# konrad-kaminski/ratelimit

Hardware: AMD Instinct MI355X
Metric: rate-limit decisions/sec (whole node) at 10M/1B keys; p99 batch latency (higher is better)
Workload: dtype u32

## Files before the change

### ratelimit_amd/csrc/rl_engine.h

```cpp
#pragma once

#include <hip/hip_runtime.h>

#include <string>

#include "../../include/ratelimit_hip.h"
#include "rl_device.h"
#include "rl_kernels.h"
#include "rl_match.h"

namespace rl {

#ifndef RL_NBUF
#define RL_NBUF 4
#endif
constexpr uint32_t NBUF = RL_NBUF;
constexpr uint32_t ERRB_RING = 2 * NBUF;
constexpr uint32_t ERRW_B0 = NBUF + 3, ERRW_WORDS = ERRW_B0 + ERRB_RING;
constexpr uint32_t PROF_RING = 8;
constexpr uint32_t PROGRESS_RING = 64;

struct HostSlot {
  uint8_t* stem = nullptr;
  uint32_t *off = nullptr, *req = nullptr, *limit = nullptr, *hits = nullptr, *rule = nullptr;
// ... 82 lines not shown
  uint32_t *d_off = nullptr, *d_req = nullptr, *d_limit = nullptr, *d_hits = nullptr, *d_rule = nullptr;
  int64_t* d_now = nullptr;
  uint8_t *d_unit = nullptr, *d_flags = nullptr, *d_code = nullptr, *d_status = nullptr;
  uint32_t *d_rem = nullptr, *d_reset = nullptr;
  unsigned long long* d_stats = nullptr;
  uint32_t* h_err = nullptr;
  uint32_t* h_long = nullptr;
  uint32_t long_recent = 0;
  int long_mode = 1;
  uint32_t* h_big = nullptr;
  uint32_t big_recent = 0;
  int big_mode = 1;
  uint32_t* h_late = nullptr;
  uint32_t late_recent = 0;
  int late_mode = 1;
  unsigned long long* h_counters = nullptr;
  std::string last_error;
  uint64_t batches = 0, decisions = 0;
  bool prof = false;
  uint32_t prof_every = 1, prof_skip = 0;
  bool prof_pending[PROF_RING] = {};
  uint32_t prof_next = 0;
  hipEvent_t ev[PROF_RING][RL_NUM_STAGES + 1] = {};
  double stage_ms[RL_NUM_STAGES] = {};
  uint64_t prof_batches = 0;
  unsigned long long* d_kt_acc = nullptr;
  double wclk_khz = 0;
  uint8_t* cfg_blob = nullptr;
  CfgDev cfg_dev{};
  bool cfg_loaded = false;
// ... 97 lines not shown
```

### ratelimit_amd/csrc/rl_engine.hip

```cpp
#include <hip/hip_runtime.h>
#include <hip/hip_ext.h>

#include <algorithm>
#include <chrono>
#include <cstdio>
#include <cstdlib>
#include <random>
#include <cstring>
#include <string>
#include <vector>

#include "../../include/ratelimit_hip.h"
#include "rl_device.h"
#include "rl_kernels.h"
#include "rl_match.h"
#include "rl_engine.h"

using namespace rl;



namespace {

thread_local std::string g_err;
// ... 130 lines not shown
    big_full = c->big_recent > 0;
    if (c->big_recent) c->big_recent--;
  }
  uint32_t* bhint = c->big_mode == 1 ? c->h_big + k : nullptr;
  bool late_full = c->late_mode == 0;
  if (c->late_mode == 1) {
    for (uint32_t j = 0; j < NBUF; j++)
      if (__atomic_load_n(&c->h_late[j], __ATOMIC_RELAXED)) {
        __atomic_store_n(&c->h_late[j], 0u, __ATOMIC_RELAXED);
        c->late_recent = 4 * NBUF;
      }
    late_full = c->late_recent > 0;
    if (c->late_recent) c->late_recent--;
  }
  uint32_t* lhint = c->late_mode == 1 ? c->h_late + k : nullptr;
  if (pipelined) {
    hipStream_t a = c->pipe[k];
    hipEvent_t* ev = prof_events(c);
    (void)hipStreamWaitEvent(a, c->b_done[k], 0);
    (void)hipStreamWaitEvent(a, c->consumed[k], 0);
    launch_stage_a(b, c->s[k], isolate, P.per_second, a, ev, hint, lng, bhint, big_full);
    if (early) launch_b_begin_early(b, o, c->s[k], restore, a, c->log_ctr);
    (void)hipStreamWaitEvent(a, c->b_table[c->last], 0);
    launch_stage_b(b, o, t, P, c->s[k], restore, a, ev, errb_prev, c->b_table[k], ev ? c->d_kt_acc : nullptr,
                   early, lhint, late_full);
    (void)hipEventRecord(c->b_done[k], a);
  } else {
    if (!st) st = c->stream;
    (void)after_batches(c, st);
    hipEvent_t* ev = prof_events(c);
    launch_stage_a(b, c->s[k], isolate, P.per_second, st, ev, hint, lng, bhint, big_full);
    if (early) launch_b_begin_early(b, o, c->s[k], restore, st, c->log_ctr);
    launch_stage_b(b, o, t, P, c->s[k], restore, st, ev, errb_prev, c->b_table[k], ev ? c->d_kt_acc : nullptr,
                   early, lhint, late_full);
    (void)hipEventRecord(c->b_done[k], st);
  }
  c->last = k;
  return k;
}

hipError_t track(Engine* c, hipStream_t st) {
  if (c->seq_sub - c->seq_done >= PROGRESS_RING) {
    const hipError_t e = hipEventSynchronize(c->done_ring[c->seq_done % PROGRESS_RING]);
    if (e != hipSuccess) return e;
    c->seq_done++;
  }
  const hipError_t e = hipEventRecord(c->done_ring[c->seq_sub % PROGRESS_RING], st);
  c->seq_sub++;
  return e;
// ... 254 lines not shown
  ok = ok && dalloc(&c->d_code, n) == hipSuccess && dalloc(&c->d_status, n) == hipSuccess &&
       dalloc(&c->d_rem, n) == hipSuccess &&
       dalloc(&c->d_reset, n) == hipSuccess;
  ok = ok && dalloc(&c->d_stats, (size_t)cfg.max_rules * RL_NUM_STATS) == hipSuccess;
  ok = ok && hipHostMalloc((void**)&c->h_err, ERRW_WORDS * sizeof(uint32_t)) == hipSuccess;
  ok = ok && hipHostMalloc((void**)&c->h_counters, 8 * sizeof(unsigned long long)) == hipSuccess;
  ok = ok && hipHostMalloc((void**)&c->h_long, NBUF * sizeof(uint32_t)) == hipSuccess;
  if (ok) memset(c->h_long, 0, NBUF * sizeof(uint32_t));
  if (const char* sl = getenv("RL_SPLIT_LONG")) c->long_mode = atoi(sl);
  ok = ok && hipHostMalloc((void**)&c->h_big, NBUF * sizeof(uint32_t)) == hipSuccess;
  if (ok) memset(c->h_big, 0, NBUF * sizeof(uint32_t));
  if (const char* bc = getenv("RL_BIG_CUE")) c->big_mode = atoi(bc);
  ok = ok && hipHostMalloc((void**)&c->h_late, NBUF * sizeof(uint32_t)) == hipSuccess;
  if (ok) memset(c->h_late, 0, NBUF * sizeof(uint32_t));
  if (const char* lc = getenv("RL_LATE_CUE")) c->late_mode = atoi(lc);
  if (!ok) return fail("gpu: device allocation failed (table_slots/arena/max_batch too large?)", c);
  ok = hipMemsetAsync(c->slots, 0, c->nslots * sizeof(Slot), c->stream) == hipSuccess &&
       hipMemsetAsync(c->log_ctr, 0, (size_t)(LOG_PARTS + 1) * LOG_CTR_STRIDE * 8, c->stream) == hipSuccess &&
       hipMemsetAsync(c->errw, 0, ERRW_WORDS * 4, c->stream) == hipSuccess &&
       hipMemsetAsync(s0.time_floor, 0, 8, c->stream) == hipSuccess &&
       hipMemsetAsync(s0.counters, 0, 64, c->stream) == hipSuccess &&
       hipMemsetAsync(c->s[0].stripes, 0, (size_t)STAT_STRIPES * STAT_LDS_RULES * RL_NUM_STATS * 8, c->stream) ==
           hipSuccess &&
       hipMemsetAsync(c->d_stem, 0, (size_t)cfg.max_stem_bytes + 64, c->stream) == hipSuccess &&
       hipStreamSynchronize(c->stream) == hipSuccess;
  for (uint32_t k = 0; k < NBUF; k++)
    ok = ok && hipEventRecord(c->b_done[k], c->stream) == hipSuccess &&
         hipEventRecord(c->b_table[k], c->stream) == hipSuccess &&
         (k == 0 || hipMemsetAsync(c->s[k].stripes, 0, (size_t)STAT_STRIPES * STAT_LDS_RULES * RL_NUM_STATS * 8,
                                   c->stream) == hipSuccess) &&
// ... 72 lines not shown
  if (c->h_base) (void)hipHostFree(c->h_base);
  const Scratch& s0 = c->s[0];
  void* bufs[] = {c->slots, c->log, c->log_ctr, c->tear, c->arena, c->arena2, c->errw, s0.stripes, s0.time_floor, s0.counters, c->d_stem, c->d_off,
                  c->d_now, c->d_req, c->d_unit, c->d_flags, c->d_limit, c->d_hits, c->d_rule, c->d_code, c->d_status,
                  c->d_rem,
                  c->d_reset, c->d_stats};
  for (void* p : bufs)
    if (p) (void)hipFree(p);
  for (uint32_t k = 1; k < NBUF; k++)
    if (c->s[k].stripes) (void)hipFree(c->s[k].stripes);
  if (c->h_err) (void)hipHostFree(c->h_err);
  if (c->h_counters) (void)hipHostFree(c->h_counters);
  if (c->h_long) (void)hipHostFree(c->h_long);
  if (c->h_big) (void)hipHostFree(c->h_big);
  if (c->h_late) (void)hipHostFree(c->h_late);
  for (void* p : {(void*)c->cfg_blob, (void*)c->mbuf})
    if (p) (void)hipFree(p);
  if (c->h_match) (void)hipHostFree(c->h_match);
  for (uint32_t k = 0; k < NBUF; k++)
    if (c->pipe[k]) (void)hipStreamDestroy(c->pipe[k]);
  delete c;
}

int eng_do_limit_async(Engine* c, const rl_batch* in, rl_result* out, void* stream) {
  if (!c || !in || !out) return set_err(c, RL_E_INVALID, "gpu: null argument");
  RQ_SETTLE(c);
  int rc = check_sizes(c, in, 0);
  if (rc) return rc;
  if ((uintptr_t)in->stem_bytes & 3u) return set_err(c, RL_E_INVALID, "gpu: stem_bytes must be 4-byte aligned");
  HIPCHK(c, hipSetDevice(c->cfg.device));
// ... 2189 lines not shown
```

### ratelimit_amd/csrc/rl_kernels.h

```cpp
#pragma once

#include <hip/hip_runtime.h>
#include <stdint.h>

#include "rl_device.h"

namespace rl {

#ifndef RL_PART_ITEMS
#define RL_PART_ITEMS 16
#endif
constexpr uint32_t PART_ITEMS = RL_PART_ITEMS, PART_TILE = 256 * PART_ITEMS;
constexpr uint32_t PART_BITS = 10, PART_DIGITS = 1u << PART_BITS;
#ifndef RL_BIG_BLOCKS
#define RL_BIG_BLOCKS 64
#endif
constexpr uint32_t BIG_BLOCKS = RL_BIG_BLOCKS;
constexpr uint32_t BIG_ITEM_BLOCKS = 256;
constexpr uint32_t BIG_HEAVY = 4;

struct BigMeta {
  uint32_t d, S, base, nchunks, item0, r, rb_heavy, db_heavy;
  uint32_t heavy[BIG_HEAVY];
};
// ... 176 lines not shown
  uint32_t* errb;
  uint32_t* errs;
  int64_t* time_floor;
  unsigned long long* counters;
  uint32_t* route_start;
  uint8_t* route_dest;
  unsigned long long* route_hash;
  uint32_t* route_hist;
  unsigned long long* r_base;
  uint32_t* woff;
  unsigned long long* wtsum;
};

void launch_stage_a(const BatchDev& b, const Scratch& s, int isolate, int per_second, hipStream_t st,
                    hipEvent_t* ev = nullptr, uint32_t* long_hint = nullptr, bool long_kernel = false,
                    uint32_t* big_hint = nullptr, bool big_full = true);
void launch_stage_b(const BatchDev& b, const OutDev& o, const TableDev& t, const Params& P, const Scratch& s,
                    int restore, hipStream_t st, hipEvent_t* ev, const uint32_t* errb_prev, hipEvent_t table_done,
                    unsigned long long* kt_acc = nullptr, bool early = false, uint32_t* late_hint = nullptr,
                    bool late_full = true);
void launch_b_begin_early(const BatchDev& b, const OutDev& o, const Scratch& s, int restore, hipStream_t st,
                          const unsigned long long* log_ctr);
void launch_unpack(const rl_batch_compact& cb, const uint8_t* buf, uint32_t* req, uint8_t* unit, uint8_t* flags,
                   uint32_t* limit, uint32_t* hits, uint32_t* rule, int64_t* now, uint32_t* err, hipStream_t st);
void launch_unpack_range(const rl_batch_compact& cb, const uint8_t* buf, uint32_t d0, uint32_t d1, uint32_t q0,
                         uint32_t q1, uint32_t* req, uint8_t* unit, uint8_t* flags, uint32_t* limit, uint32_t* hits,
                         uint32_t* rule, int64_t* now, uint32_t* err, hipStream_t st);
constexpr uint32_t TO_HOST_MAX = 6;
struct ToHost {
  const uint8_t* src[TO_HOST_MAX];
  uint8_t* dst[TO_HOST_MAX];
  uint64_t bytes[TO_HOST_MAX];
  uint32_t n;
};
void launch_to_host(const ToHost& c, hipStream_t st);
// ... 73 lines not shown
```

### ratelimit_amd/csrc/rl_kernels.hip

```cpp
#include <hip/hip_runtime.h>
#include <stdint.h>
#include <cstdlib>

#include "rl_device.h"
#include "rl_kernels.h"

#ifndef RL_ABL
#define RL_ABL 0
#endif

namespace rl {

constexpr uint32_t HASH_LDS_BYTES = 16384;

__global__ __launch_bounds__(256) void k_prepare(BatchDev b, Rec* __restrict__ rec, uint32_t* __restrict__ keys,
                                                 uint32_t* err, uint32_t* errs, int isolate,
                                                 const int64_t* time_floor, uint32_t* defer_n,
                                                 uint32_t* big_n, uint32_t* work_n, uint32_t* __restrict__ run_flags,
                                                 unsigned long long* num_runs, uint32_t* __restrict__ hit_a,
                                                 unsigned long long* __restrict__ res, uint32_t* sorted_n,
                                                 uint32_t* uniq_n) {
  __shared__ uint32_t lds[HASH_LDS_BYTES / 4 + 4];
  const uint32_t tid = threadIdx.x;
  const uint32_t i = blockIdx.x * 256 + tid;
// ... 1575 lines not shown
      }
    }
    __syncthreads();
#pragma unroll
    for (uint32_t i = 0; i < B::ITEMS; i++) {
      const uint32_t p = strip0 + i * 64 + lane;
      if (p < n) {
        kk[i] = L.k[p];
        vv[i] = L.v[p];
        hh[i] = L.h[p];
      }
    }
  }
}

template <typename B, bool FROM_LDS>
__device__ inline void bucket_segment(BucketLds<B>& L, uint32_t d, uint32_t S, uint32_t base,
                                      const uint32_t* __restrict__ sk, const uint32_t* __restrict__ sh,
                                      uint32_t* __restrict__ segsum, uint32_t* __restrict__ rid,
                                      uint32_t* __restrict__ run_start, uint32_t* __restrict__ run_end,
                                      unsigned long long* num_runs, uint32_t* __restrict__ drun) {
  constexpr uint32_t IT = B::ITEMS;
  const uint32_t tid = threadIdx.x, lane = tid & 63, wave = tid >> 6;
  auto key = [&](uint32_t p) -> uint32_t { return FROM_LDS ? L.k[p] : sk[base + p]; };
  auto hit = [&](uint32_t p) -> uint32_t { return FROM_LDS ? L.h[p] : sh[base + p]; };
  uint32_t nh = 0, nd = 0;
  for (uint32_t c0 = 0; c0 < S; c0 += B::CAP) {
    uint32_t a[IT], b[IT], c[IT];
#pragma unroll
    for (uint32_t i = 0; i < IT; i++) {
      const uint32_t p = min(c0 + i * B::THREADS + tid, S - 1);
      a[i] = key(p ? p - 1 : 0);
      b[i] = key(p);
      c[i] = key(p > 1 ? p - 2 : 0);
    }
#pragma unroll
    for (uint32_t i = 0; i < IT; i++) {
      const uint32_t p = c0 + i * B::THREADS + tid;
      nh += (p < S && (p == 0 || a[i] != b[i])) ? 1u : 0u;
      nd += (p < S && p >= 1 && a[i] == b[i] && (p == 1 || c[i] != a[i])) ? 1u : 0u;
    }
  }
  nh = block_sum(L, nh);
  nd = block_sum(L, nd);
  BK_STAMP(d, 4);
  if (tid == 0) {
    const unsigned long long old = atomicAdd(num_runs, ((unsigned long long)nd << 32) | nh);
    L.rb = (uint32_t)old;
    L.db = (uint32_t)(old >> 32);
    L.dcnt = 0;
    L.nruns = nh;
    L.carry = SegPair{0, 0};
    L.hcarry = 0;
  }
  __syncthreads();
  const uint32_t rb = L.rb;
  for (uint32_t c0 = 0; c0 < S; c0 += B::CAP) {
    const uint32_t s0 = c0 + wave * B::STRIP;
    const uint32_t ni = s0 >= S ? 0u : min(IT, (S - s0 + 63) / 64);
    SegChunk ch[IT];
    SegPair agg{0, 0};
    uint32_t hc = 0;
    uint32_t kp[IT], kq[IT], hq[IT], kpp[IT];
#pragma unroll
    for (uint32_t j = 0; j < IT; j++) {
      const uint32_t q = min(s0 + 64 * j + lane, S - 1);
      kp[j] = key(q ? q - 1 : 0);
      kq[j] = key(q);
      hq[j] = hit(q);
      kpp[j] = key(q > 1 ? q - 2 : 0);
// ... 107 lines not shown
      const uint32_t y = __shfl_up(incl, o, 64);
      if (lane >= o) incl += y;
    }
    uint32_t rank = incl - nc;
#pragma unroll
    for (uint32_t i = 0; i < R; i++)
      if (first[i] && cnt[i] >= BK_HEAVY_MIN) {
        if (rank < BK_HEAVY) L.heavy[rank] = ks[i];
        rank++;
      }
    if (lane == 63) L.nheavy = min(incl, BK_HEAVY);
  }
  __syncthreads();
}

__global__ __launch_bounds__(BkSmall::THREADS, 4) void k_bucket(
    const uint4* __restrict__ pt,
    const uint32_t* __restrict__ info, uint32_t ntiles, uint32_t* __restrict__ sk, uint32_t* __restrict__ sv,
    uint32_t* __restrict__ sh, uint32_t* __restrict__ segsum, uint32_t* __restrict__ rid,
    uint32_t* __restrict__ run_start, uint32_t* __restrict__ run_end, unsigned long long* num_runs,
    uint32_t* __restrict__ drun, BigMeta* __restrict__ meta, uint32_t* big_n, uint32_t* __restrict__ work,
    uint32_t* work_n, uint32_t* sorted_n, uint2* __restrict__ uniq, uint32_t* uniq_n, const uint32_t* err,
    uint32_t* big_hint) {
  using B = BkSmall;
  __shared__ BucketLds<B> L;
  if (*err) return;
  const uint32_t tid = threadIdx.x, lane = tid & 63, wave = tid >> 6, d = blockIdx.x;
  BK_STAMP(d, 0);
  bucket_setup(L, info, ntiles, d);
  const uint32_t S = L.S;
// ... 40 lines not shown
  }
  BK_STAMP(d, 2);
  uint32_t* ht = L.v;
  uint8_t* df = reinterpret_cast<uint8_t*>(&L.wcnt[0][0]);
  static_assert(sizeof(L.wcnt) >= B::CAP, "dup flags fit the multisplit rows");
  constexpr uint32_t HT = 2 * B::CAP, HT_SHIFT = 32 - 12;
  static_assert(HT == 1u << 12, "hash index bits");
#pragma unroll
  for (uint32_t i = 0; i < B::ITEMS; i++) {
    const uint32_t p = strip0 + i * 64 + lane;
    if (p < S) L.k[p] = kk[i];
  }
  for (uint32_t j = tid; j < HT; j += B::THREADS) ht[j] = 0xFFFFFFFFu;
  for (uint32_t j = tid; j < B::CAP / 4; j += B::THREADS) reinterpret_cast<uint32_t*>(df)[j] = 0u;
  __syncthreads();
#pragma unroll
  for (uint32_t i = 0; i < B::ITEMS; i++) {
    const uint32_t p = strip0 + i * 64 + lane;
    if (p >= S) continue;
    uint32_t h = (kk[i] * 0x9E3779B1u) >> HT_SHIFT;
    for (;;) {
      const uint32_t o = atomicCAS(&ht[h], 0xFFFFFFFFu, p);
      if (o == 0xFFFFFFFFu) break;
      if (L.k[o] == kk[i]) {
        df[p] = 1;
        df[o] = 1;
        break;
      }
      h = (h + 1) & (HT - 1);
    }
  }
  __syncthreads();
  const uint64_t lt = (1ull << lane) - 1;
  uint32_t cidx[B::ITEMS], sidx[B::ITEMS], wc = 0, ws = 0, dmask = 0, smask = 0;
#pragma unroll
  for (uint32_t i = 0; i < B::ITEMS; i++) {
    const uint32_t p = strip0 + i * 64 + lane;
    const bool dup = p < S && df[p], one = p < S && !df[p];
    const uint64_t bl = __ballot(dup), bs = __ballot(one);
    cidx[i] = wc + (uint32_t)__popcll(bl & lt);
    sidx[i] = ws + (uint32_t)__popcll(bs & lt);
    wc += (uint32_t)__popcll(bl);
    ws += (uint32_t)__popcll(bs);
    dmask |= dup ? 1u << i : 0u;
    smask |= one ? 1u << i : 0u;
  }
  if (lane == 0) {
    L.wsum[wave] = wc;
    L.lw[wave] = ws;
  }
  __syncthreads();
  uint32_t wpre = 0, M = 0, spre = 0;
#pragma unroll
  for (uint32_t w = 0; w < B::WAVES; w++) {
    wpre += w < wave ? L.wsum[w] : 0u;
    spre += w < wave ? L.lw[w] : 0u;
    M += L.wsum[w];
  }
#pragma unroll
  for (uint32_t i = 0; i < B::ITEMS; i++) {
    if (!((dmask >> i) & 1u)) continue;
    const uint32_t c = wpre + cidx[i];
    L.k[c] = kk[i];
    L.v[c] = vv[i];
    L.h[c] = hh[i];
  }
  if (tid == 0) {
    if (M) L.base_pos = atomicAdd(sorted_n, M);
    L.ub = M < S ? atomicAdd(uniq_n, S - M) : 0u;
  }
  __syncthreads();
  const uint32_t ub = L.ub + spre;
#pragma unroll
  for (uint32_t i = 0; i < B::ITEMS; i++)
    if ((smask >> i) & 1u) uniq[ub + sidx[i]] = make_uint2(vv[i], kk[i]);
  if (!M) return;
  const uint32_t base = L.base_pos;
  if (M <= 64) {
    if (wave == 0) {
      const bool v = lane < M;
      const uint32_t k = v ? L.k[lane] : 0xFFFFFFFFu, x = v ? L.v[lane] : 0u, y = v ? L.h[lane] : 0u;
      uint32_t r = 0;
      for (uint32_t j = 0; j < M; j++) {
        const uint32_t kj = __shfl(k, j, 64);
        r += (kj < k || (kj == k && j < lane)) ? 1u : 0u;
      }
      if (v) {
        L.k[r] = k;
        L.v[r] = x;
        L.h[r] = y;
      }
    }
    __syncthreads();
  } else {
#pragma unroll
    for (uint32_t i = 0; i < B::ITEMS; i++) {
      const uint32_t p = strip0 + i * 64 + lane;
      kk[i] = p < M ? L.k[p] : 0xFFFFFFFFu;
      vv[i] = p < M ? L.v[p] : 0u;
      hh[i] = p < M ? L.h[p] : 0u;
    }
    __syncthreads();
    lds_sort3(L, kk, vv, hh, M);
  }
  for (uint32_t p = tid; p < M; p += B::THREADS) {
    sk[base + p] = L.k[p];
    sv[base + p] = L.v[p];
  }
  BK_STAMP(d, 3);
  bucket_segment<B, true>(L, d, M, base, sk, sh, segsum, rid, run_start, run_end, num_runs, drun);
  BK_STAMP(d, 5);
}

template <typename B>
__device__ inline bool bucket_peel(BucketLds<B>& L, uint32_t d, uint32_t S, uint32_t base, uint32_t ntiles,
                                   const uint4* __restrict__ pt,
                                   uint32_t* __restrict__ sk,
                                   uint32_t* __restrict__ sv, uint32_t* __restrict__ sh) {
  constexpr uint32_t IT = B::ITEMS;
  const uint32_t tid = threadIdx.x, lane = tid & 63, wave = tid >> 6;
  const uint64_t lt_mask = (1ull << lane) - 1;
  if (wave == 0) {
    uint32_t p[1] = {(uint32_t)(((uint64_t)(2 * lane + 1) * S) >> 7)}, j[1];
    bucket_src(ntiles, p, j);
    const uint32_t ks = pt[j[0]].x;
// ... 566 lines not shown
      BK_STAMP(d, 1);
      if (!bucket_peel(L, d, S, base, ntiles, pt, sk, sv, sh))
        bucket_lsd(L, S, base, ntiles, pt, sk, sv, sh, ht, segsum, rid);
      bucket_segment<B, false>(L, d, S, base, sk, sh, segsum, rid, run_start, run_end, num_runs, drun);
    }
    BK_STAMP(d, 7);
    __syncthreads();
  }
}

#ifndef RL_RC_CHUNK
#define RL_RC_CHUNK 256
#endif
constexpr uint32_t RC_CHUNK = RL_RC_CHUNK;

template <typename Pred>
__device__ __attribute__((always_inline)) inline uint32_t block_compact(uint32_t lo, uint32_t hi, uint32_t* list,
                                                                        uint32_t* count, Pred pred) {
  const uint32_t lane = threadIdx.x & 63;
  if (threadIdx.x == 0) *count = 0;
  __syncthreads();
  for (uint32_t i0 = lo; i0 < hi; i0 += blockDim.x) {
    const uint32_t i = i0 + threadIdx.x;
    const bool take = i < hi && pred(i);
    const uint64_t m = __ballot(take);
    uint32_t base = 0;
    if (lane == 0 && m) base = atomicAdd(count, (uint32_t)__popcll(m));
    base = __shfl(base, 0);
    if (take) list[base + __popcll(m & ((1ull << lane) - 1))] = i;
  }
// ... 2 lines not shown
}

constexpr uint32_t SPLIT_POS_OTHER = 0xFFu, SPLIT_POS_SKIP = 0xFEu, SPLIT_POS_NOWVAR = 1u << 16;
constexpr uint32_t SPLIT_ULIST = 1024;

__global__ __launch_bounds__(256) void k_run_check(BatchDev b, SRec rec_s,
                                                   const uint32_t* __restrict__ skeys,
                                                   const uint32_t* __restrict__ rid,
                                                   const uint32_t* __restrict__ run_start,
                                                   uint32_t* __restrict__ run_end,
                                                   uint32_t* __restrict__ run_flags, uint32_t* __restrict__ defer,
                                                   uint32_t* defer_n, const uint32_t* err,
                                                   const unsigned long long* num_runs, unsigned long long* split,
                                                   const uint32_t* sorted_n, uint32_t* __restrict__ pos_unit,
                                                   uint32_t* __restrict__ pos_hits, uint2* __restrict__ uniq,
                                                   uint32_t* uniq_n, uint32_t* long_runs, uint32_t* __restrict__ keys0) {
  __shared__ uint32_t s_list[RC_CHUNK], s_cnt;
  if (blockIdx.x == 0 && threadIdx.x == 0) {
    split[0] = 0;
    split[1] = *num_runs;
    long_runs[0] = 0;
  }
  if (*err) return;
  const uint32_t sn = *sorted_n;
  for (uint32_t q0 = blockIdx.x * RC_CHUNK; q0 < min(blockIdx.x * RC_CHUNK + RC_CHUNK, sn); q0 += blockDim.x) {
    const uint32_t q = q0 + threadIdx.x;
    const uint32_t k = q < sn ? skeys[q] : 0u;
    const bool one = q < sn && (q == 0 || skeys[q - 1] != k) && (q + 1 >= sn || skeys[q + 1] != k);
    const uint64_t m = __ballot(one);
    if (!m) continue;
    const uint32_t lane = threadIdx.x & 63, leader = (uint32_t)__ffsll((unsigned long long)m) - 1;
    uint32_t at = 0;
    if (lane == leader) at = atomicAdd(uniq_n, (uint32_t)__popcll(m));
    at = __shfl(at, leader, 64) + (uint32_t)__popcll(m & ((1ull << lane) - 1));
    if (one) uniq[at] = make_uint2(rec_s.sv[q], k);
  }
  const uint32_t lo = max(blockIdx.x * RC_CHUNK, 1u), hi = min(blockIdx.x * RC_CHUNK + RC_CHUNK, sn);
  if (lo >= hi) return;
  const uint32_t cnt = block_compact(lo, hi, s_list, &s_cnt, [&](uint32_t q) { return skeys[q - 1] == skeys[q]; });
  refine_totals(b);
  Rec* rec = const_cast<Rec*>(rec_s.rec);
#pragma unroll 1
  for (uint32_t j = threadIdx.x; j < cnt; j += blockDim.x) {
    const uint32_t q = s_list[j];
    const uint32_t r = rid[q];
    const uint32_t p = run_start[r];
    const uint32_t eq = rec_s.sv[q], ep = rec_s.sv[p];
    const Rec x = rec[eq], y = rec[ep];
    const bool skip = (rec_flags(x) | rec_flags(y)) & FLAG_SKIP;
    const bool same_stem = !skip && x.hlo == y.hlo && (x.lu & 0xFFFFu) == (y.lu & 0xFFFFu) &&
                           key_equal(key_of(b, x), key_of(b, y));
    if (!same_stem && !skip && q == p + 1 && run_end[r] == q + 1) {
      run_end[r] = p;
      const uint32_t at = atomicAdd(uniq_n, 2u);
      uniq[at] = make_uint2(ep, skeys[q]);
      uniq[at + 1] = make_uint2(eq, skeys[q]);
      continue;
    }
    keys0[eq] = KEY_DUP;
    if (q == p + 1) keys0[ep] = KEY_DUP;
    const bool same = same_stem && rec_unit(x) == rec_unit(y);
    pos_unit[q] = (rec_unit(x) << 8) | (skip ? SPLIT_POS_SKIP : !same_stem ? SPLIT_POS_OTHER : 0u) |
                  (x.now != y.now ? SPLIT_POS_NOWVAR : 0u);
    pos_hits[q] = x.hits > 1 ? x.hits : 1u;
    uint32_t f = 0;
    if (!same)
      f = RUN_MULTI | (same_stem ? RUN_UNITS | ((1u << (rec_unit(x) - 1)) << RUN_UMASK_SHIFT) : RUN_STEMS);
    if (x.now != y.now) {
      const uint32_t d = div_of(rec_unit(x));
      f |= (same && x.now / d != y.now / d) ? RUN_SLOW | RUN_NOWVAR : RUN_NOWVAR;
    }
// ... 111 lines not shown
#define RL_SPLIT_LONG_BLOCKS 8
#endif
#ifndef RL_SPLIT_THREADS
#define RL_SPLIT_THREADS 256
#endif
constexpr uint32_t SPLIT_THREADS = RL_SPLIT_THREADS;

struct UniqList {
  uint2* list;
  uint32_t* n;
  const uint32_t* skeys;
  uint32_t* keys0;
  __device__ inline void single(uint32_t e, uint32_t p) const {
    const uint32_t k = skeys[p];
    keys0[e] = k;
    list[atomicAdd(n, 1u)] = make_uint2(e, k);
  }
};

template <uint32_t NT, uint32_t ST>
__device__ __attribute__((always_inline)) inline void split_long_body(uint32_t j, uint32_t r, uint32_t p, uint32_t L, BatchDev b,
                                                          SRec rec_s, uint32_t* svals, uint32_t* segsum,
                                                          uint32_t* __restrict__ rid, uint32_t* __restrict__ run_start,
                                                          uint32_t* __restrict__ run_end,
                                                          uint32_t* __restrict__ run_flags, uint32_t* __restrict__ defer,
                                                          unsigned long long* num_runs, unsigned long long* split,
                                                          uint32_t* __restrict__ drun, uint32_t drun_cap, uint32_t* grp,
                                                          uint32_t* rank, uint32_t* __restrict__ pos_hits,
                                                          uint32_t* __restrict__ hnew, int per_second, uint32_t rfl,
                                                          const UniqList& uq) {
  constexpr uint32_t NW = NT / 64;
// ... 577 lines not shown
        if (!f) v += carry;
        if (in) segsum[p + k] = v;
        carry = __shfl(v, 63, 64);
      }
    }
    if (tid < G) {
      const uint32_t id = s_id[tid];
      run_start[id] = p + s_base[tid];
      run_end[id] = p + s_base[tid] + s_cnt[tid];
      run_flags[id] = split_group_flags(s_plan, tid, s_fl[tid]);
    }
    if (tid == 0) defer[j] = DEFER_DONE;
  }
}

#ifndef RL_UNIQ_DENSE
#define RL_UNIQ_DENSE 3
#endif
__device__ __attribute__((always_inline)) inline void unique_body(uint32_t blk, BatchDev b, TableDev t, Params P, const Rec* __restrict__ rec,
                                                const uint32_t* __restrict__ keys0,
                                                const uint2* __restrict__ uniq, const uint32_t* uniq_n,
                                                unsigned long long* __restrict__ res,
                                                uint32_t* __restrict__ defer1, uint32_t* defer1_n,
                                                unsigned long long* stats, unsigned long long* stripes, uint32_t* err,
                                                uint32_t* errs, int restore, const uint32_t* errb_prev) {
  __shared__ uint32_t s_err, s_nu, s_cnt, s_list[256];
  if (threadIdx.x == 0) {
    s_err = __hip_atomic_load(err, __ATOMIC_RELAXED, __HIP_MEMORY_SCOPE_AGENT) | (errb_prev ? *errb_prev : 0u);
    s_nu = *uniq_n;
  }
  __syncthreads();
  const uint32_t nu = s_nu;
  const bool by_list = (uint64_t)nu * 4 < (uint64_t)b.n * RL_UNIQ_DENSE;
  const uint32_t lo = blk * 256, hi = min(lo + 256, by_list ? nu : b.n);
  if (s_err || lo >= hi) return;
  refine_totals(b);
  uint32_t* ferr = P.isolate ? errs : err;
  const bool use_lds = !restore && b.n_rules <= LDS_RULES;
  stats_block_begin(use_lds, b.n_rules);
  StatAcc acc{use_lds, stats};
  LaneStats L;
  L.reset();
  auto single = [&](uint32_t i) { return keys0[i] != KEY_DUP && !((rec[i].lu >> 24) & FLAG_SKIP); };
  bool act;
  uint32_t i, key = 0;
  if (by_list) {
    const uint32_t pos = lo + threadIdx.x;
    const uint2 ent = pos < hi ? uniq[pos] : make_uint2(0u, 0u);
// ... 1385 lines not shown
  const uint32_t d = div_of(unit[i]);
  reset[i] = d - (uint32_t)(now[i] % d);
  unsigned long long* s = deltas + (size_t)i * RL_NUM_STATS;
  s[RL_STAT_TOTAL_HITS] = 0;
  s[RL_STAT_OVER_LIMIT] = r.d_over;
  s[RL_STAT_NEAR_LIMIT] = r.d_near;
  s[RL_STAT_OVER_LIMIT_WITH_LOCAL_CACHE] = r.d_lc;
  s[RL_STAT_WITHIN_LIMIT] = r.d_within;
  s[RL_STAT_SHADOW_MODE] = r.d_shadow;
  lc_set[i] = r.set_lc;
}

static inline uint32_t cdiv(uint64_t a, uint64_t b) { return (uint32_t)((a + b - 1) / b); }

void launch_stage_a(const BatchDev& b, const Scratch& s, int isolate, int per_second, hipStream_t st,
                    hipEvent_t* ev, uint32_t* long_hint, bool long_kernel, uint32_t* big_hint, bool big_full) {
  const uint32_t g0 = cdiv(b.n > b.n_req ? b.n : b.n_req, 256);
  if (ev) (void)hipEventRecord(ev[0], st);
  if (g0)
    k_prepare<<<g0, 256, 0, st>>>(b, s.rec, s.keys[0], s.err, s.errs, isolate, s.time_floor, s.defer_n, s.big_n,
                                  s.work_n, s.run_flags, s.runs64, s.hit_a, s.res, s.sorted_n, s.uniq_n);
  if (ev) (void)hipEventRecord(ev[1], st);
  const uint32_t ptiles = cdiv(b.n, PART_TILE);
  if (b.n)
    k_part<<<ptiles, 256, 0, st>>>(s.keys[0], b.wire ? s.hit_a : b.hits, s.tile, b.n, ptiles, s.part_info, s.err);
  if (ev) (void)hipEventRecord(ev[2], st);
  if (b.n) {
    const size_t seg_lds = (2ull * ptiles + 1) * 4;
    k_bucket<<<PART_DIGITS, BkSmall::THREADS, seg_lds, st>>>(s.tile, s.part_info, ptiles,
                                                             s.keys[1], s.vals[0], s.hits_s, s.segsum, s.rid,
                                                             s.run_start, s.run_end, s.runs64, s.drun, s.big_meta, s.big_n,
                                                             s.big_work, s.work_n, s.sorted_n, s.uniq, s.uniq_n,
                                                             s.err, big_hint);
#ifndef RL_EXP_NO_BIG
    const uint32_t gi = big_full ? BIG_ITEM_BLOCKS : 1u, gb = big_full ? BIG_BLOCKS : 1u;
    k_big_count<<<gi, BkSmall::THREADS, seg_lds, st>>>(s.tile, s.part_info, ptiles,
                                                                    s.big_meta, s.big_work, s.work_n, s.big_cnt,
                                                                    s.err);
    k_big_place<<<gi, BkSmall::THREADS, seg_lds, st>>>(
        s.tile, s.part_info, ptiles, s.big_meta, s.big_work, s.work_n, s.big_cnt, s.keys[1],
        s.vals[0], s.hits_s, s.segsum, s.rid, s.run_start, s.run_end, s.drun, s.err);
    k_bucket_big<<<gb, BkBig::THREADS, seg_lds, st>>>(s.tile, s.part_info, ptiles,
                                                              s.keys[1], s.vals[0], s.hits_s, s.hit_t, s.segsum,
                                                              s.rid, s.run_start, s.run_end, s.runs64, s.drun, s.big_meta,
                                                              s.big_n, s.big_cnt, s.err);
#endif
    k_run_check<<<cdiv(b.n, RC_CHUNK), 256, 0, st>>>(b, SRec{s.rec, s.vals[0]}, s.keys[1], s.rid, s.run_start,
                                                s.run_end, s.run_flags, s.defer, s.defer_n, s.err, s.runs64, s.split,
                                                s.sorted_n, s.grp, s.hit_t, s.uniq, s.uniq_n, s.long_runs, s.keys[0]);
#ifndef RL_EXP_NO_SPLIT
    k_split<<<SPLIT_BLOCKS, SPLIT_THREADS, 0, st>>>(b, SRec{s.rec, s.vals[0]}, s.vals[0], s.segsum, s.rid, s.run_start,
                                          s.run_end, s.run_flags, s.defer, s.defer_n, s.runs64, s.split, s.drun,
                                          b.n / 2 + BIG_HEAVY * PART_DIGITS, s.grp, s.lead, s.hit_t, s.vals[1], s.err,
                                          per_second, UniqList{s.uniq, s.uniq_n, s.keys[1], s.keys[0]}, s.long_runs, long_hint,
                                          long_kernel ? 1 : 0);
#endif
#if RL_SPLIT_LONG_THREADS
    if (long_kernel)
      k_split_long<<<RL_SPLIT_LONG_BLOCKS, RL_SPLIT_LONG_THREADS, 0, st>>>(
          b, SRec{s.rec, s.vals[0]}, s.vals[0], s.segsum, s.rid, s.run_start, s.run_end, s.run_flags, s.defer,
          s.runs64, s.split, s.drun, b.n / 2 + BIG_HEAVY * PART_DIGITS, s.grp, s.lead, s.hit_t, s.vals[1], s.err,
          per_second, UniqList{s.uniq, s.uniq_n, s.keys[1], s.keys[0]}, s.long_runs);
#endif
  }
}

#ifndef RL_LATE_FAST_BLOCKS
#define RL_LATE_FAST_BLOCKS 0
#endif
constexpr uint32_t LATE_SCAN_BLOCKS = 4;
void launch_b_begin_early(const BatchDev& b, const OutDev& o, const Scratch& s, int restore, hipStream_t st,
                          const unsigned long long* log_ctr) {
  const uint32_t m = restore ? 0u : b.n_rules * RL_NUM_STATS;
  const uint32_t gb = m ? (cdiv(m, 256) < 64 ? cdiv(m, 256) : 64) : 1;
  k_b_begin<<<gb, 256, 0, st>>>(s.err, s.errb, nullptr, s.defer2_n, s.defer1_n, o.stats, m, s.fast_blk,
                                cdiv(b.n, 256 * 32), log_ctr, s.log_epoch);
}

void launch_stage_b(const BatchDev& b, const OutDev& o, const TableDev& t, const Params& P, const Scratch& s,
                    int restore, hipStream_t st, hipEvent_t* ev, const uint32_t* errb_prev, hipEvent_t table_done,
                    unsigned long long* kt_acc, bool early, uint32_t* late_hint, bool late_full) {
  const uint32_t m = restore ? 0u : b.n_rules * RL_NUM_STATS;
  const uint32_t gb = m ? (cdiv(m, 256) < 64 ? cdiv(m, 256) : 64) : 1;
  if (!early)
    k_b_begin<<<gb, 256, 0, st>>>(s.err, s.errb, errb_prev, s.defer2_n, s.defer1_n, o.stats, m, s.fast_blk,
                                  cdiv(b.n, 256 * 32), t.log_ctr, s.log_epoch);
  else if (!b.n)
    k_b_begin<<<1, 256, 0, st>>>(s.errb, s.errb, errb_prev, s.defer2_n, s.defer1_n, o.stats, 0, s.fast_blk, 0,
                                 nullptr, nullptr);
  if (b.n) {
    const uint32_t g = cdiv(b.n, 256);
    const size_t lds = (!restore && b.n_rules <= LDS_RULES) ? (size_t)b.n_rules * RL_NUM_STATS * 8 : 0;
    const SRec rs{s.rec, s.vals[0]};
    if (ev) (void)hipEventRecord(ev[3], st);
    const uint32_t g_runs = cdiv(b.n / 2 + BIG_HEAVY * PART_DIGITS, 256);
    k_table<<<g_runs + g, 256, lds, st>>>(g_runs, b, t, P, rs, s.keys[1], s.vals[0], s.res, s.run_start, s.run_end,
                                         s.run_flags, s.run_state, s.run_alias, s.rid, s.run_f, s.runs64, s.drun,
                                         s.defer2, s.defer2_n,
                                         s.keys[0], s.defer1, s.defer1_n, o.stats, s.stripes, s.errb, s.errs, restore,
                                         s.fast_blk, s.uniq, s.uniq_n, kt_acc ? s.kt_blk : nullptr,
                                         early ? errb_prev : nullptr);
    if (ev) (void)hipEventRecord(ev[4], st);
    if (!restore && P.lc_en)
      k_fast_over<<<g, 256, 0, st>>>(s.sorted_n, rs, s.segsum, s.rid, s.run_flags, s.run_state, s.run_f, s.errb);
#ifndef RL_EXP_NO_LATE
    const uint32_t gl = restore ? 0u : !late_full ? LATE_SCAN_BLOCKS
                                     : (RL_LATE_FAST_BLOCKS && g > RL_LATE_FAST_BLOCKS ? RL_LATE_FAST_BLOCKS : g);
    k_late<<<RUNS_GENERAL_LATE_BLOCKS + gl, 256, lds, st>>>(
        b, t, P, rs, s.keys[1], s.vals[0], s.res, s.run_start, s.run_end, s.defer, s.defer_n, s.defer2, s.defer2_n,
        s.grp, s.lead, s.gmask,
        s.keys[0], s.defer1, s.defer1_n, s.segsum, s.rid, s.run_flags, s.run_state, s.run_alias, s.run_f, o.stats,
        s.stripes, s.errb,
        s.errs, restore, s.fast_blk, s.sorted_n, late_hint, late_full ? 0 : 1);
#endif
    if (table_done) (void)hipEventRecord(table_done, st);
// ... 89 lines not shown
```

Before: 6.023 billion.

## Skip building the unique-key list when a device hint says it is unused

Adds a host-polled hint, following the existing cue pattern, that records when the unique-key list would actually be used for the dense/list choice. When the hint is off, the bucket, run-check and split kernels skip building the uniq list and the unique pass walks all keys. Separately, k_bucket now counts runs during its hash-insert pass and reserves run slots with a single atomic, so bucket_segment can skip its counting sweep and block reduction. The risk is extra template variants and a lagging heuristic: list building turns back on only a few batches after the device flags it.

Measured after the change: 6.190 billion (median of 6 runs). +2.8%, better.

```diff
diff --git a/ratelimit_amd/csrc/rl_engine.h b/ratelimit_amd/csrc/rl_engine.h
--- a/ratelimit_amd/csrc/rl_engine.h
+++ b/ratelimit_amd/csrc/rl_engine.h
@@ -120,6 +120,9 @@
   uint32_t* h_late = nullptr;
   uint32_t late_recent = 0;
   int late_mode = 1;
+  uint32_t* h_list = nullptr;
+  uint32_t list_recent = 0;
+  int list_mode = 1;
   unsigned long long* h_counters = nullptr;
   std::string last_error;
   uint64_t batches = 0, decisions = 0;
diff --git a/ratelimit_amd/csrc/rl_engine.hip b/ratelimit_amd/csrc/rl_engine.hip
--- a/ratelimit_amd/csrc/rl_engine.hip
+++ b/ratelimit_amd/csrc/rl_engine.hip
@@ -168,25 +168,36 @@
     if (c->late_recent) c->late_recent--;
   }
   uint32_t* lhint = c->late_mode == 1 ? c->h_late + k : nullptr;
+  bool list_on = c->list_mode == 0;
+  if (c->list_mode == 1) {
+    for (uint32_t j = 0; j < NBUF; j++)
+      if (__atomic_load_n(&c->h_list[j], __ATOMIC_RELAXED)) {
+        __atomic_store_n(&c->h_list[j], 0u, __ATOMIC_RELAXED);
+        c->list_recent = 4 * NBUF;
+      }
+    list_on = c->list_recent > 0;
+    if (c->list_recent) c->list_recent--;
+  }
+  uint32_t* uhint = c->list_mode == 1 ? c->h_list + k : nullptr;
   if (pipelined) {
     hipStream_t a = c->pipe[k];
     hipEvent_t* ev = prof_events(c);
     (void)hipStreamWaitEvent(a, c->b_done[k], 0);
     (void)hipStreamWaitEvent(a, c->consumed[k], 0);
-    launch_stage_a(b, c->s[k], isolate, P.per_second, a, ev, hint, lng, bhint, big_full);
+    launch_stage_a(b, c->s[k], isolate, P.per_second, a, ev, hint, lng, bhint, big_full, uhint, list_on);
     if (early) launch_b_begin_early(b, o, c->s[k], restore, a, c->log_ctr);
     (void)hipStreamWaitEvent(a, c->b_table[c->last], 0);
     launch_stage_b(b, o, t, P, c->s[k], restore, a, ev, errb_prev, c->b_table[k], ev ? c->d_kt_acc : nullptr,
-                   early, lhint, late_full);
+                   early, lhint, late_full, list_on);
     (void)hipEventRecord(c->b_done[k], a);
   } else {
     if (!st) st = c->stream;
     (void)after_batches(c, st);
     hipEvent_t* ev = prof_events(c);
-    launch_stage_a(b, c->s[k], isolate, P.per_second, st, ev, hint, lng, bhint, big_full);
+    launch_stage_a(b, c->s[k], isolate, P.per_second, st, ev, hint, lng, bhint, big_full, uhint, list_on);
     if (early) launch_b_begin_early(b, o, c->s[k], restore, st, c->log_ctr);
     launch_stage_b(b, o, t, P, c->s[k], restore, st, ev, errb_prev, c->b_table[k], ev ? c->d_kt_acc : nullptr,
-                   early, lhint, late_full);
+                   early, lhint, late_full, list_on);
     (void)hipEventRecord(c->b_done[k], st);
   }
   c->last = k;
@@ -471,6 +482,9 @@
   ok = ok && hipHostMalloc((void**)&c->h_late, NBUF * sizeof(uint32_t)) == hipSuccess;
   if (ok) memset(c->h_late, 0, NBUF * sizeof(uint32_t));
   if (const char* lc = getenv("RL_LATE_CUE")) c->late_mode = atoi(lc);
+  ok = ok && hipHostMalloc((void**)&c->h_list, NBUF * sizeof(uint32_t)) == hipSuccess;
+  if (ok) memset(c->h_list, 0, NBUF * sizeof(uint32_t));
+  if (const char* uc = getenv("RL_LIST_CUE")) c->list_mode = atoi(uc);
   if (!ok) return fail("gpu: device allocation failed (table_slots/arena/max_batch too large?)", c);
   ok = hipMemsetAsync(c->slots, 0, c->nslots * sizeof(Slot), c->stream) == hipSuccess &&
        hipMemsetAsync(c->log_ctr, 0, (size_t)(LOG_PARTS + 1) * LOG_CTR_STRIDE * 8, c->stream) == hipSuccess &&
@@ -573,6 +587,7 @@
   if (c->h_long) (void)hipHostFree(c->h_long);
   if (c->h_big) (void)hipHostFree(c->h_big);
   if (c->h_late) (void)hipHostFree(c->h_late);
+  if (c->h_list) (void)hipHostFree(c->h_list);
   for (void* p : {(void*)c->cfg_blob, (void*)c->mbuf})
     if (p) (void)hipFree(p);
   if (c->h_match) (void)hipHostFree(c->h_match);
diff --git a/ratelimit_amd/csrc/rl_kernels.h b/ratelimit_amd/csrc/rl_kernels.h
--- a/ratelimit_amd/csrc/rl_kernels.h
+++ b/ratelimit_amd/csrc/rl_kernels.h
@@ -214,11 +214,12 @@
 
 void launch_stage_a(const BatchDev& b, const Scratch& s, int isolate, int per_second, hipStream_t st,
                     hipEvent_t* ev = nullptr, uint32_t* long_hint = nullptr, bool long_kernel = false,
-                    uint32_t* big_hint = nullptr, bool big_full = true);
+                    uint32_t* big_hint = nullptr, bool big_full = true, uint32_t* list_hint = nullptr,
+                    bool list_on = true);
 void launch_stage_b(const BatchDev& b, const OutDev& o, const TableDev& t, const Params& P, const Scratch& s,
                     int restore, hipStream_t st, hipEvent_t* ev, const uint32_t* errb_prev, hipEvent_t table_done,
                     unsigned long long* kt_acc = nullptr, bool early = false, uint32_t* late_hint = nullptr,
-                    bool late_full = true);
+                    bool late_full = true, bool list_on = true);
 void launch_b_begin_early(const BatchDev& b, const OutDev& o, const Scratch& s, int restore, hipStream_t st,
                           const unsigned long long* log_ctr);
 void launch_unpack(const rl_batch_compact& cb, const uint8_t* buf, uint32_t* req, uint8_t* unit, uint8_t* flags,
diff --git a/ratelimit_amd/csrc/rl_kernels.hip b/ratelimit_amd/csrc/rl_kernels.hip
--- a/ratelimit_amd/csrc/rl_kernels.hip
+++ b/ratelimit_amd/csrc/rl_kernels.hip
@@ -1613,7 +1613,7 @@
   }
 }
 
-template <typename B, bool FROM_LDS>
+template <typename B, bool FROM_LDS, bool PRE = false>
 __device__ inline void bucket_segment(BucketLds<B>& L, uint32_t d, uint32_t S, uint32_t base,
                                       const uint32_t* __restrict__ sk, const uint32_t* __restrict__ sh,
                                       uint32_t* __restrict__ segsum, uint32_t* __restrict__ rid,
@@ -1624,7 +1624,7 @@
   auto key = [&](uint32_t p) -> uint32_t { return FROM_LDS ? L.k[p] : sk[base + p]; };
   auto hit = [&](uint32_t p) -> uint32_t { return FROM_LDS ? L.h[p] : sh[base + p]; };
   uint32_t nh = 0, nd = 0;
-  for (uint32_t c0 = 0; c0 < S; c0 += B::CAP) {
+  for (uint32_t c0 = 0; !PRE && c0 < S; c0 += B::CAP) {
     uint32_t a[IT], b[IT], c[IT];
 #pragma unroll
     for (uint32_t i = 0; i < IT; i++) {
@@ -1640,19 +1640,21 @@
       nd += (p < S && p >= 1 && a[i] == b[i] && (p == 1 || c[i] != a[i])) ? 1u : 0u;
     }
   }
-  nh = block_sum(L, nh);
-  nd = block_sum(L, nd);
-  BK_STAMP(d, 4);
-  if (tid == 0) {
-    const unsigned long long old = atomicAdd(num_runs, ((unsigned long long)nd << 32) | nh);
-    L.rb = (uint32_t)old;
-    L.db = (uint32_t)(old >> 32);
-    L.dcnt = 0;
-    L.nruns = nh;
-    L.carry = SegPair{0, 0};
-    L.hcarry = 0;
-  }
-  __syncthreads();
+  if constexpr (!PRE) {
+    nh = block_sum(L, nh);
+    nd = block_sum(L, nd);
+    BK_STAMP(d, 4);
+    if (tid == 0) {
+      const unsigned long long old = atomicAdd(num_runs, ((unsigned long long)nd << 32) | nh);
+      L.rb = (uint32_t)old;
+      L.db = (uint32_t)(old >> 32);
+      L.dcnt = 0;
+      L.nruns = nh;
+      L.carry = SegPair{0, 0};
+      L.hcarry = 0;
+    }
+    __syncthreads();
+  }
   const uint32_t rb = L.rb;
   for (uint32_t c0 = 0; c0 < S; c0 += B::CAP) {
     const uint32_t s0 = c0 + wave * B::STRIP;
@@ -1790,6 +1792,10 @@
   __syncthreads();
 }
 
+#ifndef RL_BK_EARLY
+#define RL_BK_EARLY 1
+#endif
+template <bool LIST>
 __global__ __launch_bounds__(BkSmall::THREADS, 4) void k_bucket(
     const uint4* __restrict__ pt,
     const uint32_t* __restrict__ info, uint32_t ntiles, uint32_t* __restrict__ sk, uint32_t* __restrict__ sv,
@@ -1860,6 +1866,7 @@
   for (uint32_t j = tid; j < HT; j += B::THREADS) ht[j] = 0xFFFFFFFFu;
   for (uint32_t j = tid; j < B::CAP / 4; j += B::THREADS) reinterpret_cast<uint32_t*>(df)[j] = 0u;
   __syncthreads();
+  uint32_t win = 0;
 #pragma unroll
   for (uint32_t i = 0; i < B::ITEMS; i++) {
     const uint32_t p = strip0 + i * 64 + lane;
@@ -1867,7 +1874,10 @@
     uint32_t h = (kk[i] * 0x9E3779B1u) >> HT_SHIFT;
     for (;;) {
       const uint32_t o = atomicCAS(&ht[h], 0xFFFFFFFFu, p);
-      if (o == 0xFFFFFFFFu) break;
+      if (o == 0xFFFFFFFFu) {
+        win |= 1u << i;
+        break;
+      }
       if (L.k[o] == kk[i]) {
         df[p] = 1;
         df[o] = 1;
@@ -1878,30 +1888,37 @@
   }
   __syncthreads();
   const uint64_t lt = (1ull << lane) - 1;
-  uint32_t cidx[B::ITEMS], sidx[B::ITEMS], wc = 0, ws = 0, dmask = 0, smask = 0;
+  uint32_t cidx[B::ITEMS], sidx[LIST ? B::ITEMS : 1], wc = 0, ws = 0, wr = 0, dmask = 0, smask = 0;
 #pragma unroll
   for (uint32_t i = 0; i < B::ITEMS; i++) {
     const uint32_t p = strip0 + i * 64 + lane;
-    const bool dup = p < S && df[p], one = p < S && !df[p];
-    const uint64_t bl = __ballot(dup), bs = __ballot(one);
+    const bool dup = p < S && df[p];
+    const uint64_t bl = __ballot(dup);
     cidx[i] = wc + (uint32_t)__popcll(bl & lt);
-    sidx[i] = ws + (uint32_t)__popcll(bs & lt);
     wc += (uint32_t)__popcll(bl);
-    ws += (uint32_t)__popcll(bs);
     dmask |= dup ? 1u << i : 0u;
-    smask |= one ? 1u << i : 0u;
+    if (RL_BK_EARLY) wr += (uint32_t)__popcll(__ballot(dup && ((win >> i) & 1u)));
+    if constexpr (LIST) {
+      const bool one = p < S && !df[p];
+      const uint64_t bs = __ballot(one);
+      sidx[i] = ws + (uint32_t)__popcll(bs & lt);
+      ws += (uint32_t)__popcll(bs);
+      smask |= one ? 1u << i : 0u;
+    }
   }
   if (lane == 0) {
     L.wsum[wave] = wc;
-    L.lw[wave] = ws;
+    L.sh[wave] = wr;
+    if (LIST) L.lw[wave] = ws;
   }
   __syncthreads();
-  uint32_t wpre = 0, M = 0, spre = 0;
+  uint32_t wpre = 0, M = 0, spre = 0, nh = 0;
 #pragma unroll
   for (uint32_t w = 0; w < B::WAVES; w++) {
     wpre += w < wave ? L.wsum[w] : 0u;
-    spre += w < wave ? L.lw[w] : 0u;
+    if (LIST) spre += w < wave ? L.lw[w] : 0u;
     M += L.wsum[w];
+    nh += L.sh[w];
   }
 #pragma unroll
   for (uint32_t i = 0; i < B::ITEMS; i++) {
@@ -1911,17 +1928,23 @@
     L.v[c] = vv[i];
     L.h[c] = hh[i];
   }
+  uint32_t r_base = 0;
+  unsigned long long r_runs = 0;
   if (tid == 0) {
-    if (M) L.base_pos = atomicAdd(sorted_n, M);
-    L.ub = M < S ? atomicAdd(uniq_n, S - M) : 0u;
+    if (M) {
+      r_base = atomicAdd(sorted_n, M);
+      if (RL_BK_EARLY) r_runs = atomicAdd(num_runs, ((unsigned long long)nh << 32) | nh);
+    }
+    if constexpr (LIST) L.ub = M < S ? atomicAdd(uniq_n, S - M) : 0u;
   }
   __syncthreads();
-  const uint32_t ub = L.ub + spre;
-#pragma unroll
-  for (uint32_t i = 0; i < B::ITEMS; i++)
-    if ((smask >> i) & 1u) uniq[ub + sidx[i]] = make_uint2(vv[i], kk[i]);
+  if constexpr (LIST) {
+    const uint32_t ub = L.ub + spre;
+#pragma unroll
+    for (uint32_t i = 0; i < B::ITEMS; i++)
+      if ((smask >> i) & 1u) uniq[ub + sidx[i]] = make_uint2(vv[i], kk[i]);
+  }
   if (!M) return;
-  const uint32_t base = L.base_pos;
   if (M <= 64) {
     if (wave == 0) {
       const bool v = lane < M;
@@ -1937,7 +1960,6 @@
         L.h[r] = y;
       }
     }
-    __syncthreads();
   } else {
 #pragma unroll
     for (uint32_t i = 0; i < B::ITEMS; i++) {
@@ -1949,12 +1971,26 @@
     __syncthreads();
     lds_sort3(L, kk, vv, hh, M);
   }
+  if (tid == 0) {
+    L.base_pos = r_base;
+    if (RL_BK_EARLY) {
+      L.rb = (uint32_t)r_runs;
+      L.db = (uint32_t)(r_runs >> 32);
+      L.dcnt = 0;
+      L.nruns = nh;
+      L.carry = SegPair{0, 0};
+      L.hcarry = 0;
+    }
+  }
+  __syncthreads();
+  const uint32_t base = L.base_pos;
   for (uint32_t p = tid; p < M; p += B::THREADS) {
     sk[base + p] = L.k[p];
     sv[base + p] = L.v[p];
   }
   BK_STAMP(d, 3);
-  bucket_segment<B, true>(L, d, M, base, sk, sh, segsum, rid, run_start, run_end, num_runs, drun);
+  [[clang::always_inline]] bucket_segment<B, true, RL_BK_EARLY != 0>(L, d, M, base, sk, sh, segsum, rid, run_start,
+                                                                     run_end, num_runs, drun);
   BK_STAMP(d, 5);
 }
 
@@ -2551,6 +2587,10 @@
 #endif
 constexpr uint32_t RC_CHUNK = RL_RC_CHUNK;
 
+#ifndef RL_UNIQ_DENSE
+#define RL_UNIQ_DENSE 3
+#endif
+
 template <typename Pred>
 __device__ __attribute__((always_inline)) inline uint32_t block_compact(uint32_t lo, uint32_t hi, uint32_t* list,
                                                                         uint32_t* count, Pred pred) {
@@ -2583,7 +2623,8 @@
                                                    const unsigned long long* num_runs, unsigned long long* split,
                                                    const uint32_t* sorted_n, uint32_t* __restrict__ pos_unit,
                                                    uint32_t* __restrict__ pos_hits, uint2* __restrict__ uniq,
-                                                   uint32_t* uniq_n, uint32_t* long_runs, uint32_t* __restrict__ keys0) {
+                                                   uint32_t* uniq_n, uint32_t* long_runs, uint32_t* __restrict__ keys0,
+                                                   int list_on, uint32_t* list_hint) {
   __shared__ uint32_t s_list[RC_CHUNK], s_cnt;
   if (blockIdx.x == 0 && threadIdx.x == 0) {
     split[0] = 0;
@@ -2592,7 +2633,9 @@
   }
   if (*err) return;
   const uint32_t sn = *sorted_n;
-  for (uint32_t q0 = blockIdx.x * RC_CHUNK; q0 < min(blockIdx.x * RC_CHUNK + RC_CHUNK, sn); q0 += blockDim.x) {
+  if (list_hint && blockIdx.x == 0 && threadIdx.x == 0 && (uint64_t)(b.n - min(sn, b.n)) * 4 < (uint64_t)b.n * RL_UNIQ_DENSE)
+    *list_hint = 1u;
+  for (uint32_t q0 = blockIdx.x * RC_CHUNK; list_on && q0 < min(blockIdx.x * RC_CHUNK + RC_CHUNK, sn); q0 += blockDim.x) {
     const uint32_t q = q0 + threadIdx.x;
     const uint32_t k = q < sn ? skeys[q] : 0u;
     const bool one = q < sn && (q == 0 || skeys[q - 1] != k) && (q + 1 >= sn || skeys[q + 1] != k);
@@ -2621,9 +2664,11 @@
                            key_equal(key_of(b, x), key_of(b, y));
     if (!same_stem && !skip && q == p + 1 && run_end[r] == q + 1) {
       run_end[r] = p;
-      const uint32_t at = atomicAdd(uniq_n, 2u);
-      uniq[at] = make_uint2(ep, skeys[q]);
-      uniq[at + 1] = make_uint2(eq, skeys[q]);
+      if (list_on) {
+        const uint32_t at = atomicAdd(uniq_n, 2u);
+        uniq[at] = make_uint2(ep, skeys[q]);
+        uniq[at + 1] = make_uint2(eq, skeys[q]);
+      }
       continue;
     }
     keys0[eq] = KEY_DUP;
@@ -2765,7 +2810,7 @@
   __device__ inline void single(uint32_t e, uint32_t p) const {
     const uint32_t k = skeys[p];
     keys0[e] = k;
-    list[atomicAdd(n, 1u)] = make_uint2(e, k);
+    if (list) list[atomicAdd(n, 1u)] = make_uint2(e, k);
   }
 };
 
@@ -3373,9 +3418,6 @@
   }
 }
 
-#ifndef RL_UNIQ_DENSE
-#define RL_UNIQ_DENSE 3
-#endif
 __device__ __attribute__((always_inline)) inline void unique_body(uint32_t blk, BatchDev b, TableDev t, Params P, const Rec* __restrict__ rec,
                                                 const uint32_t* __restrict__ keys0,
                                                 const uint2* __restrict__ uniq, const uint32_t* uniq_n,
@@ -3384,13 +3426,14 @@
                                                 unsigned long long* stats, unsigned long long* stripes, uint32_t* err,
                                                 uint32_t* errs, int restore, const uint32_t* errb_prev) {
   __shared__ uint32_t s_err, s_nu, s_cnt, s_list[256];
+  const bool list_on = uniq_n != nullptr;
   if (threadIdx.x == 0) {
     s_err = __hip_atomic_load(err, __ATOMIC_RELAXED, __HIP_MEMORY_SCOPE_AGENT) | (errb_prev ? *errb_prev : 0u);
-    s_nu = *uniq_n;
+    s_nu = list_on ? *uniq_n : 0u;
   }
   __syncthreads();
   const uint32_t nu = s_nu;
-  const bool by_list = (uint64_t)nu * 4 < (uint64_t)b.n * RL_UNIQ_DENSE;
+  const bool by_list = list_on && (uint64_t)nu * 4 < (uint64_t)b.n * RL_UNIQ_DENSE;
   const uint32_t lo = blk * 256, hi = min(lo + 256, by_list ? nu : b.n);
   if (s_err || lo >= hi) return;
   refine_totals(b);
@@ -4806,7 +4849,8 @@
 static inline uint32_t cdiv(uint64_t a, uint64_t b) { return (uint32_t)((a + b - 1) / b); }
 
 void launch_stage_a(const BatchDev& b, const Scratch& s, int isolate, int per_second, hipStream_t st,
-                    hipEvent_t* ev, uint32_t* long_hint, bool long_kernel, uint32_t* big_hint, bool big_full) {
+                    hipEvent_t* ev, uint32_t* long_hint, bool long_kernel, uint32_t* big_hint, bool big_full,
+                    uint32_t* list_hint, bool list_on) {
   const uint32_t g0 = cdiv(b.n > b.n_req ? b.n : b.n_req, 256);
   if (ev) (void)hipEventRecord(ev[0], st);
   if (g0)
@@ -4819,11 +4863,9 @@
   if (ev) (void)hipEventRecord(ev[2], st);
   if (b.n) {
     const size_t seg_lds = (2ull * ptiles + 1) * 4;
-    k_bucket<<<PART_DIGITS, BkSmall::THREADS, seg_lds, st>>>(s.tile, s.part_info, ptiles,
-                                                             s.keys[1], s.vals[0], s.hits_s, s.segsum, s.rid,
-                                                             s.run_start, s.run_end, s.runs64, s.drun, s.big_meta, s.big_n,
-                                                             s.big_work, s.work_n, s.sorted_n, s.uniq, s.uniq_n,
-                                                             s.err, big_hint);
+    (list_on ? k_bucket<true> : k_bucket<false>)<<<PART_DIGITS, BkSmall::THREADS, seg_lds, st>>>(
+        s.tile, s.part_info, ptiles, s.keys[1], s.vals[0], s.hits_s, s.segsum, s.rid, s.run_start, s.run_end,
+        s.runs64, s.drun, s.big_meta, s.big_n, s.big_work, s.work_n, s.sorted_n, s.uniq, s.uniq_n, s.err, big_hint);
 #ifndef RL_EXP_NO_BIG
     const uint32_t gi = big_full ? BIG_ITEM_BLOCKS : 1u, gb = big_full ? BIG_BLOCKS : 1u;
     k_big_count<<<gi, BkSmall::THREADS, seg_lds, st>>>(s.tile, s.part_info, ptiles,
@@ -4839,12 +4881,13 @@
 #endif
     k_run_check<<<cdiv(b.n, RC_CHUNK), 256, 0, st>>>(b, SRec{s.rec, s.vals[0]}, s.keys[1], s.rid, s.run_start,
                                                 s.run_end, s.run_flags, s.defer, s.defer_n, s.err, s.runs64, s.split,
-                                                s.sorted_n, s.grp, s.hit_t, s.uniq, s.uniq_n, s.long_runs, s.keys[0]);
+                                                s.sorted_n, s.grp, s.hit_t, s.uniq, s.uniq_n, s.long_runs, s.keys[0],
+                                                list_on ? 1 : 0, list_hint);
 #ifndef RL_EXP_NO_SPLIT
     k_split<<<SPLIT_BLOCKS, SPLIT_THREADS, 0, st>>>(b, SRec{s.rec, s.vals[0]}, s.vals[0], s.segsum, s.rid, s.run_start,
                                           s.run_end, s.run_flags, s.defer, s.defer_n, s.runs64, s.split, s.drun,
                                           b.n / 2 + BIG_HEAVY * PART_DIGITS, s.grp, s.lead, s.hit_t, s.vals[1], s.err,
-                                          per_second, UniqList{s.uniq, s.uniq_n, s.keys[1], s.keys[0]}, s.long_runs, long_hint,
+                                          per_second, UniqList{list_on ? s.uniq : nullptr, s.uniq_n, s.keys[1], s.keys[0]}, s.long_runs, long_hint,
                                           long_kernel ? 1 : 0);
 #endif
 #if RL_SPLIT_LONG_THREADS
@@ -4852,7 +4895,7 @@
       k_split_long<<<RL_SPLIT_LONG_BLOCKS, RL_SPLIT_LONG_THREADS, 0, st>>>(
           b, SRec{s.rec, s.vals[0]}, s.vals[0], s.segsum, s.rid, s.run_start, s.run_end, s.run_flags, s.defer,
           s.runs64, s.split, s.drun, b.n / 2 + BIG_HEAVY * PART_DIGITS, s.grp, s.lead, s.hit_t, s.vals[1], s.err,
-          per_second, UniqList{s.uniq, s.uniq_n, s.keys[1], s.keys[0]}, s.long_runs);
+          per_second, UniqList{list_on ? s.uniq : nullptr, s.uniq_n, s.keys[1], s.keys[0]}, s.long_runs);
 #endif
   }
 }
@@ -4871,7 +4914,7 @@
 
 void launch_stage_b(const BatchDev& b, const OutDev& o, const TableDev& t, const Params& P, const Scratch& s,
                     int restore, hipStream_t st, hipEvent_t* ev, const uint32_t* errb_prev, hipEvent_t table_done,
-                    unsigned long long* kt_acc, bool early, uint32_t* late_hint, bool late_full) {
+                    unsigned long long* kt_acc, bool early, uint32_t* late_hint, bool late_full, bool list_on) {
   const uint32_t m = restore ? 0u : b.n_rules * RL_NUM_STATS;
   const uint32_t gb = m ? (cdiv(m, 256) < 64 ? cdiv(m, 256) : 64) : 1;
   if (!early)
@@ -4890,7 +4933,7 @@
                                          s.run_flags, s.run_state, s.run_alias, s.rid, s.run_f, s.runs64, s.drun,
                                          s.defer2, s.defer2_n,
                                          s.keys[0], s.defer1, s.defer1_n, o.stats, s.stripes, s.errb, s.errs, restore,
-                                         s.fast_blk, s.uniq, s.uniq_n, kt_acc ? s.kt_blk : nullptr,
+                                         s.fast_blk, s.uniq, list_on ? s.uniq_n : nullptr, kt_acc ? s.kt_blk : nullptr,
                                          early ? errb_prev : nullptr);
     if (ev) (void)hipEventRecord(ev[4], st);
     if (!restore && P.lc_en)
```
